# wenbowen123/iros20-6d-pose-tracking

Measured on AMD Instinct MI355X. Metric: RGB-D pair inferences/sec (176x176), higher is better.
Workload: dtype f32; 1 GPU; configs[1]: batch=64 synthetic 176x176 RGB-D pairs per GPU, random-init Se3TrackNet (reference state_dict surface), stage=full; pairs_per_gpu=64, global_batch=64, stage=full, frames=resident in HBM

## Files before the change

### iros20-6d-pose-tracking_amd/csrc/api.cpp

```cpp
#include <cmath>
#include <thread>
#include <type_traits>
#include <cstdio>
#include <cstdlib>
#include <chrono>
#include <cstring>
#include <map>
#include <mutex>
#include <set>
#include <string>
#include <vector>

#include "hip_buffers.h"
#include "pose_align_plan.h"
#include "pose_errors_plan.h"
#include "pose_grid_plan.h"
#include "pose_search_plan.h"
#include "se3tn_internal.h"
#include "tex_pyramid.h"
#include "track_plan.h"
#include "weights.h"

using namespace se3tn;

// ... 17 lines not shown
struct GraphKey {
  const void *A, *B, *trans, *rot, *poseA, *poseB, *blob;
  int layout;
  InferConfig cfg;
  bool operator==(const GraphKey& o) const { return std::memcmp(this, &o, sizeof(GraphKey)) == 0; }
};
struct GraphEntry {
  GraphKey key;
  hipGraphExec_t exec = nullptr;
  InferPlan plan;
};
static_assert(std::is_trivially_copyable<GraphEntry>::value, "the graph cache moves its entries as bytes (GraphKey is compared as bytes)");

struct se3tn_ctx {
  int device = -1, max_batch = 0;
  TensorMap tensors;
  std::vector<float> packed;
  DeviceBuf<float> blob_owned;
  const float* blob = nullptr;
  BlobLayout L;
  DeviceBuf<float> inA, inB;
  DeviceBuf<float> stem;
  DeviceBuf<float> pool, t64, q64;
  DeviceBuf<float> ab, ab_t;
  DeviceBuf<float> head, head_t;
  DeviceBuf<float> head_f;
  unsigned written = 0;
  InferPlan plan;
  DeviceBuf<float> logits;
  DeviceBuf<float> fcpart;
  bool keep_intermediates = false;
  int auto_tile_override[2] = {0, 0};
  int gemmp = -1;
  bool wino_fuse = true;
  DeviceBuf<float> part;
  int tail_parts_ch = 16;
  bool tail_parts = true;
  bool small_kernels = true;
  int wino_min_batch = SE3TN_WINOGRAD_DEFAULT_MIN_BATCH;
  int wino_tile = SE3TN_WINOGRAD_DEFAULT_TILE;
  int wino_tile_derived = 0;
  DeviceBuf<float> wino_u[4];
  DeviceBuf<float> wino_u6[4];
  const float* wino6_blob = nullptr;
  DeviceBuf<float> wino_v, wino_m;
  const float* wino_blob = nullptr;
  int wino64_min_batch = SE3TN_TRUNK_WINOGRAD_DEFAULT_MIN_BATCH;
  int wino64_min_fill = SE3TN_TRUNK_WINOGRAD_DEFAULT_MIN_FILL;
  int num_cus = 256;
  DeviceBuf<float> wino64_u[4];
  const float* wino64_blob = nullptr;
  SplitLayout SL;
  DeviceBuf<float> split_w;
  const float* split_blob = nullptr;
  DeviceBuf<float> wino_us[4];
  DeviceBuf<float> wino_usc[4];
  const float* wino_us_blob = nullptr;
  int wino_us_tile = 0;
  int prec = SE3TN_PREC_F32;
  int offset_rule = SE3TN_OFFSET_RULE_NUMPY1;
  int raster_sub_bits = 4;
  PinnedBuf<uint8_t> trk_host; DeviceBuf<uint8_t> trk_dev; size_t trk_bytes = 0;
  PinnedBuf<uint8_t> trk_out;
  int tb_cap = 0;
  size_t tb_stage_bytes = 0;
  PinnedBuf<uint8_t> tb_inst_host; DeviceBuf<uint8_t> tb_inst_dev;
// ... 268 lines not shown
    d = c->ps_dev.get();
    return SE3TN_OK;
  }
  int upload(size_t bytes) const {
    HIPCHK(hipMemcpyAsync(d, h, bytes, hipMemcpyHostToDevice, st));
    return SE3TN_OK;
  }
  int finish(size_t at, size_t bytes) const {
    HIPCHK(hipMemcpyAsync(h + at, d + at, bytes, hipMemcpyDeviceToHost, st));
    HIPCHK(hipStreamSynchronize(st));
    return SE3TN_OK;
  }
  template <class T> T* dev(size_t at) const { return reinterpret_cast<T*>(d + at); }
};

extern "C" {

const char* se3tn_version(void) { return "se3tracknet-gfx950 0.6.0 (blob v7)"; }
const char* se3tn_last_error(void) { return g_err.c_str(); }

int se3tn_create(int device, int max_batch, se3tn_ctx** out) {
  if (!out || max_batch < 1) return fail(SE3TN_E_ARG, "se3tn_create: bad argument");
  if (max_batch > SE3TN_MAX_BATCH_LIMIT)
    return fail(SE3TN_E_ARG, "se3tn_create: max_batch " + std::to_string(max_batch) + " exceeds SE3TN_MAX_BATCH_LIMIT (" +
                                 std::to_string(SE3TN_MAX_BATCH_LIMIT) + "): run larger sets as several calls");
  se3tn_ctx* c = new se3tn_ctx();
  c->device = device;
  c->max_batch = max_batch;
  c->L = blob_layout();
  c->SL = split_layout();
  if (const char* e = std::getenv("SE3TN_WINOGRAD_AUTO_TILE_AB2")) c->auto_tile_override[0] = (std::atoi(e) == 4 || std::atoi(e) == 6) ? std::atoi(e) : 0;
  if (const char* e = std::getenv("SE3TN_WINOGRAD_AUTO_TILE_HEADS")) c->auto_tile_override[1] = (std::atoi(e) == 4 || std::atoi(e) == 6) ? std::atoi(e) : 0;
  if (const char* e = std::getenv("SE3TN_WINO_GEMMP")) c->gemmp = std::atoi(e) != 0 ? 1 : 0;
  if (const char* e = std::getenv("SE3TN_WINOGRAD_FUSE")) c->wino_fuse = std::atoi(e) != 0;
  if (const char* e = std::getenv("SE3TN_TRUNK_WINOGRAD")) c->wino64_min_batch = std::atoi(e);
  if (const char* e = std::getenv("SE3TN_TRUNK_WINOGRAD_FILL")) c->wino64_min_fill = std::atoi(e);
  for (int i = 0; i < 8; ++i) { c->mean[i] = 0.0; c->stdv[i] = 1.0; }
  if (device >= 0) {
    hipDeviceProp_t prop;
    hipError_t e = hipGetDeviceProperties(&prop, device);
    if (e != hipSuccess) { delete c; return hipfail(e, "hipGetDeviceProperties"); }
    if (std::strncmp(prop.gcnArchName, "gfx950", 6) != 0) {
      std::string a = prop.gcnArchName;
      delete c;
      return fail(SE3TN_E_DEVICE, "device is " + a + ", this library is built for gfx950 only");
    }
    if (prop.multiProcessorCount > 0) c->num_cus = prop.multiProcessorCount;
    e = hipSetDevice(device);
    if (e != hipSuccess) { delete c; return hipfail(e, "hipSetDevice"); }
    const size_t mb = (size_t)max_batch;
    auto padded = [&](int s, int ch) { return (mb * (s + 2) * (s + 2) + PAD_SLACK_PX) * ch; };
    struct { DeviceBuf<float>* p; size_t words; bool zero; } bufs[] = {
        {&c->inA, (mb * IN_P + IN_SLACK_ROWS) * IN_P * 4, true},
        {&c->inB, (mb * IN_P + IN_SLACK_ROWS) * IN_P * 4, true},
        {&c->stem, mb * S1 * S1 * 128, false}, {&c->pool, padded(S2, 128), true},
        {&c->t64, padded(S2, 128), true},      {&c->q64, padded(S2, 128), true},
        {&c->ab, padded(S3, 256), true},       {&c->ab_t, padded(S3, 256), true},
        {&c->head, padded(S4, 1024), true},    {&c->head_t, padded(S4, 1024), true},
        {&c->head_f, padded(S4, 1024), true},
        {&c->logits, mb * 6, true},           {&c->fcpart, mb * 192, true}};
    for (auto& b : bufs) {
      e = b.p->alloc(b.words, b.zero);
      if (e != hipSuccess) { delete c; return hipfail(e, "hipMalloc(workspace)"); }
    }
    e = c->part.alloc((size_t)16 * 1024 * 121 * 16);
    if (e == hipSuccess) e = c->tail_arrive.alloc(c->max_batch, true);
// ... 278 lines not shown
  if (fast) {
    a.fast = 1;
    a.overflow = c->overflow.get();
    a.w = c->split_w.get() + c->SL.conv_ws[r.id];
    a.wscale = c->split_w.get() + c->SL.conv_sc[r.id];
  }
  a.res = tensor_ptr(c, r.res, fast); a.out = tensor_ptr(c, r.out, fast);
  a.part = c->part.get(); a.part_bytes = c->part.count() * sizeof(float);
  a.in_ld = r.in.ld; a.res_ld = r.res.ld; a.out_ld = r.out.ld;
  a.H = r.hin; a.W = r.hin; a.Ho = (r.hin - 1) / r.stride + 1; a.Wo = a.Ho;
  a.M = n * a.Ho * a.Wo;
  a.groups = s.groups;
  a.in_gs = r.in.gs; a.res_gs = r.res.gs; a.out_gs = r.out.gs; a.bias_gs = s.cout;
  a.w_gs = (long long)conv3_words(s.cin, s.cout);
  if (ip) {
    a.per_img = 1;
    std::memcpy(a.img_off, ip->off, sizeof(a.img_off));
  }
}
static void fill_wino_args(se3tn_ctx* c, const ConvRow& r, int tile, int n, const float* W, bool split, WinoArgs& w) {
  const Conv3& s = conv_specs()[r.id];
  const int ws = wino_slot(r.id);
  w = WinoArgs{};
  w.in = tensor_ptr(c, r.in, split); w.bias = W + c->L.conv_b[r.id]; w.res = tensor_ptr(c, r.res, split); w.out = tensor_ptr(c, r.out, split);
  w.U = tile == 6 ? c->wino_u6[ws].get() : c->wino_u[ws].get();
  w.V = c->wino_v.get(); w.Mw = c->wino_m.get();
  w.in_ld = r.in.ld; w.res_ld = r.res.ld; w.out_ld = r.out.ld;
  w.m = tile; w.nf = (tile + 2) * (tile + 2);
  w.H = r.hin; w.W = r.hin; w.th = (r.hin + tile - 1) / tile; w.tw = w.th;
  w.n = n; w.T = n * w.th * w.tw;
  w.C = s.cin; w.Cout = s.cout; w.groups = s.groups;
  w.in_gs = r.in.gs; w.res_gs = r.res.gs; w.out_gs = r.out.gs; w.bias_gs = s.cout;
  w.u_gs = (long long)w.nf * s.cin * s.cout;
  if (split) {
    w.split = 1;
    w.U = c->wino_us[ws].get(); w.uscale = c->wino_usc[ws].get();
    w.overflow = c->overflow.get();
  }
}

static int infer_launch(se3tn_ctx* c, const float* A, const float* B, int n, int layout, float* trans, float* rot,
                        const double* poseA, double* poseB, void* stream);

int se3tn_enable_graphs(se3tn_ctx* c, int on) {
  if (!c || c->device < 0) return fail(SE3TN_E_ARG, "se3tn_enable_graphs: no device context");
  c->use_graphs = on != 0;
  return SE3TN_OK;
}

static int infer_graph_or_launch(se3tn_ctx* c, const float* A, const float* B, int n, int layout, float* trans, float* rot,
                                 const double* poseA, double* poseB, void* stream);

int se3tn_infer(se3tn_ctx* c, const float* A, const float* B, int n, int layout, float* trans, float* rot,
                const double* poseA, double* poseB, void* stream) {
  if (c && c->rearm_counters && c->device >= 0 && !stream_is_capturing((hipStream_t)stream)) {
    if (c->tail_arrive) HIPCHK(hipMemsetAsync(c->tail_arrive.get(), 0, sizeof(int) * c->max_batch, (hipStream_t)stream));
    c->rearm_counters = false;
  }
  const int rc = infer_graph_or_launch(c, A, B, n, layout, trans, rot, poseA, poseB, stream);
  if (rc != SE3TN_OK && rc != SE3TN_E_ARG && rc != SE3TN_E_STATE && c) c->rearm_counters = true;
  return rc;
}

static int infer_graph_or_launch(se3tn_ctx* c, const float* A, const float* B, int n, int layout, float* trans, float* rot,
                                 const double* poseA, double* poseB, void* stream) {
  if (!c || !c->use_graphs || c->prof || stream == nullptr)
// ... 1572 lines not shown
```

### iros20-6d-pose-tracking_amd/csrc/se3tn_internal.h

```cpp
#pragma once
#include <hip/hip_runtime.h>
#include <stddef.h>
#include <stdint.h>

#include "../../include/se3tracknet.h"
#include "infer_plan.h"

namespace se3tn {

struct BlobLayout {
  size_t stem_w;
  size_t stem_b;
  size_t conv_w[NUM_CONV3];
  size_t conv_b[NUM_CONV3];
  size_t fc_w;
  size_t fc_b;
  size_t total;
};

constexpr int HEADER_WORDS = 64;
constexpr uint32_t BLOB_MAGIC = 0x53453354u;
constexpr uint32_t BLOB_VERSION = 7;

struct SplitLayout {
// ... 67 lines not shown
  int groups;
  int in_gs, res_gs, out_gs, bias_gs;
  long long w_gs;
  float* part;
  size_t part_bytes;
  int slices;
  int reserved[2];
  const float* wscale;
  int* overflow;
  int fast;
  int per_img = 0;
  long long img_off[SMALL_MAX_IMG] = {};
};

struct WinoArgs {
  const float* in;
  const float* U;
  const float* bias;
  const float* res;
  float* out;
  float* V;
  float* Mw;
  int in_ld, res_ld, out_ld;
  int H, W;
  int m, nf;
  int th, tw;
  int n, T;
  int C, Cout, groups;
  int in_gs, res_gs, out_gs, bias_gs;
  long long u_gs;
  int split;
  const float* uscale;
  int* overflow;
};

struct TailArgs {
  const float* fc_w;
  const float* fc_b;
  float* logits;
  float* fcpart;
  float* trans;
  float* rot;
  const double* poseA;
  double* poseB;
  double tn, rn;
};

struct CropArgs {
  static constexpr int MAX = 64;
  se3tn_crop c[MAX];
  double mean[8], stdv[8];
  float* out;
  float* out2;
  int n_first;
  int n;
  int padded;
  int split;
  int offset_rule;
  int* overflow;
  const double* norm = nullptr;
  uint8_t* raw_rgb = nullptr;
  uint16_t* raw_depth = nullptr;
};

static_assert(sizeof(CropArgs) <= 4096, "CropArgs travels as kernel arguments: HIP's limit is 4 KB");

// ... 212 lines not shown
```

### iros20-6d-pose-tracking_amd/csrc/wino_mfma.hip

```cpp
#include "mfma_common.h"
#include "pose_device.h"

#ifndef WINO4_VEC
#define WINO4_VEC 2
#endif
#ifndef WINO_MID_CS_AB
#define WINO_MID_CS_AB 32
#endif
#ifndef WINO_MID_CS_H
#define WINO_MID_CS_H 32
#endif

#ifdef SE3TN_GEMMP_TRACE
__device__ unsigned long long se3tn_gemmp_trace[8 * 64 * 5];
extern "C" int se3tn_debug_gemmp_trace(void* host_out, size_t bytes) {
  return (int)hipMemcpyFromSymbol(host_out, HIP_SYMBOL(se3tn_gemmp_trace), bytes, 0, hipMemcpyDeviceToHost);
}
#define GP_STAMP(K, I) if (blockIdx.x == 0 && lane == 0 && (K) < 64) ::se3tn_gemmp_trace[(wid * 64 + (K)) * 5 + (I)] = __builtin_amdgcn_s_memtime();
#else
#define GP_STAMP(K, I)
#endif
#ifdef SE3TN_WG_TRACE
__device__ unsigned long long se3tn_wg_trace[8 * 4096];
extern "C" int se3tn_debug_wg_trace(void* host_out, size_t bytes, int clear) {
  if (clear) {
    void* p = nullptr;
    if (hipGetSymbolAddress(&p, HIP_SYMBOL(se3tn_wg_trace)) != hipSuccess) return 1;
    return (int)hipMemset(p, 0, sizeof(unsigned long long) * 8 * 4096);
  }
  return (int)hipMemcpyFromSymbol(host_out, HIP_SYMBOL(se3tn_wg_trace), bytes, 0, hipMemcpyDeviceToHost);
}
#endif

namespace se3tn {
// ... 59 lines not shown
  const hv h = *reinterpret_cast<const hv*>(p_);
  const hv l = *reinterpret_cast<const hv*>(p_ + 64);
#pragma unroll
  for (int e = 0; e < VEC; ++e) o[e] = (float)h[e] + (float)l[e];
}
template <int VEC>
__device__ __forceinline__ bool store_split_vec(float* base, size_t row, int ld, int c, const float (&v)[VEC]) {
  unsigned char* p_ = reinterpret_cast<unsigned char*>(base) + split_byte_off(row, ld, c);
  typedef _Float16 hv __attribute__((ext_vector_type(VEC)));
  hv h, l;
  bool bad = false;
#pragma unroll
  for (int e = 0; e < VEC; ++e) {
    h[e] = (_Float16)v[e];
    l[e] = (_Float16)(v[e] - (float)h[e]);
    bad |= !(fabsf(v[e]) <= 65000.f);
  }
  *reinterpret_cast<hv*>(p_) = h;
  *reinterpret_cast<hv*>(p_ + 64) = l;
  return bad;
}

struct TileId { int t, cv, n, ty, tx; };
__device__ __forceinline__ TileId tile_of(int idx, int cvn, int th, int tw) {
  TileId r;
  r.cv = idx % cvn; r.t = idx / cvn;
  const int tpi = th * tw;
  r.n = r.t / tpi;
  const int rem = r.t - r.n * tpi;
  r.ty = rem / tw; r.tx = rem - r.ty * tw;
  return r;
}

template <int M, int VEC, int SP = 0>
__global__ __launch_bounds__(256) void wino_input_kernel(const WinoArgs a) {
  constexpr int N = M + 2;
  typedef typename VecT<VEC>::type vec;
  const int cvn = a.C / VEC;
  const int idx = blockIdx.x * 256 + threadIdx.x;
  if (idx >= a.T * cvn) return;
  const int g = blockIdx.y;
  const TileId id = tile_of(idx, cvn, a.th, a.tw);
  const int Hp = a.H + 2, Wp = a.W + 2;
  const float* __restrict__ src = a.in + (size_t)g * a.in_gs + (SP ? 0 : id.cv * VEC);
  float bt[N][N][VEC];
  if constexpr (M == 6) {
    static_assert(SP == 0, "F(6x6) is a float32 path");
#pragma unroll
    for (int s = 0; s < N; ++s) {
      float dc[N][VEC];
      const int X = M * id.tx + s;
#pragma unroll
      for (int r = 0; r < N; ++r) {
        const int Y = M * id.ty + r;
        vec v;
        if (Y < Hp && X < Wp) v = *reinterpret_cast<const vec*>(src + (size_t)((id.n * Hp + Y) * Wp + X) * a.in_ld);
        else __builtin_memset(&v, 0, sizeof(v));
        __builtin_memcpy(dc[r], &v, sizeof(v));
      }
#pragma unroll
      for (int i = 0; i < N; ++i)
#pragma unroll
        for (int e = 0; e < VEC; ++e) {
          float acc = 0.f;
          bool first = true;
#pragma unroll
          for (int r = 0; r < N; ++r) axpy(acc, wino_bt<M>(i, r), dc[r][e], first);
          bt[i][s][e] = acc;
        }
    }
  } else {
  float d[N][N][VEC];
#pragma unroll
  for (int r = 0; r < N; ++r)
#pragma unroll
    for (int s = 0; s < N; ++s) {
      const int Y = M * id.ty + r, X = M * id.tx + s;
      if (SP) {
        if (Y < Hp && X < Wp) load_split_vec<VEC>(src, (size_t)((id.n * Hp + Y) * Wp + X), a.in_ld, id.cv * VEC, d[r][s]);
        else for (int e = 0; e < VEC; ++e) d[r][s][e] = 0.f;
        continue;
      }
      vec v;
      if (Y < Hp && X < Wp) v = *reinterpret_cast<const vec*>(src + (size_t)((id.n * Hp + Y) * Wp + X) * a.in_ld);
      else __builtin_memset(&v, 0, sizeof(v));
      __builtin_memcpy(d[r][s], &v, sizeof(v));
    }
#pragma unroll
  for (int i = 0; i < N; ++i)
#pragma unroll
    for (int s = 0; s < N; ++s)
#pragma unroll
      for (int e = 0; e < VEC; ++e) {
        float acc = 0.f;
        bool first = true;
#pragma unroll
        for (int r = 0; r < N; ++r) axpy(acc, wino_bt<M>(i, r), d[r][s][e], first);
        bt[i][s][e] = acc;
      }
  }
  float* __restrict__ dst = a.V + ((size_t)g * a.nf * a.T + id.t) * a.C + (SP ? 0 : id.cv * VEC);
  const size_t fs = (size_t)a.T * a.C;
  bool bad = false;
#pragma unroll
  for (int i = 0; i < N; ++i)
#pragma unroll
    for (int j = 0; j < N; ++j) {
      float o[VEC];
#pragma unroll
      for (int e = 0; e < VEC; ++e) {
        float acc = 0.f;
        bool first = true;
#pragma unroll
        for (int s = 0; s < N; ++s) axpy(acc, wino_bt<M>(j, s), bt[i][s][e], first);
        o[e] = acc;
      }
      if (SP) {
        bad |= store_split_vec<VEC>(dst + (size_t)(N * i + j) * fs, 0, a.C, id.cv * VEC, o);
        continue;
      }
      vec v;
      __builtin_memcpy(&v, o, sizeof(v));
      *reinterpret_cast<vec*>(dst + (size_t)(N * i + j) * fs) = v;
    }
  if (SP && bad) atomicOr(a.overflow, 1);
}

template <int M, int VEC, int EPI, int SP = 0>
__global__ __launch_bounds__(256) void wino_output_kernel(const WinoArgs a) {
  constexpr int N = M + 2;
  typedef typename VecT<VEC>::type vec;
  const int cvn = a.Cout / VEC;
  const int idx = blockIdx.x * 256 + threadIdx.x;
  if (idx >= a.T * cvn) return;
  const int g = blockIdx.y;
  const TileId id = tile_of(idx, cvn, a.th, a.tw);
  const int Hp = a.H + 2, Wp = a.W + 2;
  const float* __restrict__ src = a.Mw + ((size_t)g * a.nf * a.T + id.t) * a.Cout + id.cv * VEC;
  const size_t fs = (size_t)a.T * a.Cout;
  float rr[M][M][VEC];
  if constexpr (EPI == 1 && SP == 0) {
    const float* __restrict__ res0 = a.res + (size_t)g * a.res_gs + id.cv * VEC;
#pragma unroll
    for (int i = 0; i < M; ++i)
#pragma unroll
      for (int j = 0; j < M; ++j) {
        int oy = M * id.ty + i, ox = M * id.tx + j;
        oy = oy < a.H ? oy : a.H - 1; ox = ox < a.W ? ox : a.W - 1;
        const vec v = *reinterpret_cast<const vec*>(res0 + (size_t)((id.n * Hp + oy + 1) * Wp + ox + 1) * a.res_ld);
        __builtin_memcpy(rr[i][j], &v, sizeof(v));
      }
  }
  float u[M][N][VEC];
#pragma unroll
  for (int s = 0; s < N; ++s) {
    float m[N][VEC];
#pragma unroll
    for (int r = 0; r < N; ++r) {
      const vec v = *reinterpret_cast<const vec*>(src + (size_t)(N * r + s) * fs);
      __builtin_memcpy(m[r], &v, sizeof(v));
    }
#pragma unroll
    for (int i = 0; i < M; ++i)
#pragma unroll
      for (int e = 0; e < VEC; ++e) {
        float acc = 0.f;
        bool first = true;
#pragma unroll
        for (int r = 0; r < N; ++r) axpy(acc, wino_at<M>(i, r), m[r][e], first);
        u[i][s][e] = acc;
      }
  }
  float b[VEC];
  {
    const vec v = *reinterpret_cast<const vec*>(a.bias + (size_t)g * a.bias_gs + id.cv * VEC);
    __builtin_memcpy(b, &v, sizeof(v));
  }
  const float* __restrict__ res = (EPI == 1) ? a.res + (size_t)g * a.res_gs + (SP ? 0 : id.cv * VEC) : nullptr;
  float* __restrict__ out = a.out + (size_t)g * a.out_gs + (SP ? 0 : id.cv * VEC);
  bool bad = false;
  if constexpr (SP == 0) __builtin_amdgcn_s_waitcnt(0x0F70);
#pragma unroll
  for (int i = 0; i < M; ++i)
#pragma unroll
    for (int j = 0; j < M; ++j) {
      const int oy = M * id.ty + i, ox = M * id.tx + j;
      if (oy >= a.H || ox >= a.W) continue;
      const size_t pix = (size_t)((id.n * Hp + oy + 1) * Wp + ox + 1);
      float r[VEC];
      if (EPI == 1) {
        if (SP) {
          load_split_vec<VEC>(res, pix, a.res_ld, id.cv * VEC, r);
// ... 39 lines not shown
  double gg[N][3];
#pragma unroll
  for (int i = 0; i < N; ++i)
#pragma unroll
    for (int s = 0; s < 3; ++s) gg[i][s] = wino_g<M>(i, 0) * g[0][s] + wino_g<M>(i, 1) * g[1][s] + wino_g<M>(i, 2) * g[2][s];
  const size_t fs = (size_t)cout * 32;
  float* dst = U + ((size_t)ch * N * N * cout + co) * 32 + k;
#pragma unroll
  for (int i = 0; i < N; ++i)
#pragma unroll
    for (int j = 0; j < N; ++j)
      dst[(size_t)(N * i + j) * fs] = (float)(gg[i][0] * wino_g<M>(j, 0) + gg[i][1] * wino_g<M>(j, 1) + gg[i][2] * wino_g<M>(j, 2));
}

template <int CIN, int WM, int WN, int PT, int CT, int MM = MM_F32>
__global__ __launch_bounds__(256, 2) void wino_gemm_kernel(const WinoArgs a) {
  constexpr int BM = WM * PT * 32, BN = WN * CT * 32;
  constexpr int NCH = CIN / 32;
  constexpr int BUF = (BM + BN) * 32;
  static_assert(WM * WN == 4, "4 waves");
  extern __shared__ __attribute__((aligned(16))) float smem[];

  const int tid = threadIdx.x;
  const int lane = tid & 63;
  const int wid = __builtin_amdgcn_readfirstlane(tid >> 6);
  const int wm = wid / WN, wn = wid % WN;
  const int l31 = lane & 31, hh = lane >> 5;

  const int panels = a.Cout / BN, mtiles = (a.T + BM - 1) / BM;
  const int nt = blockIdx.x % panels, rest = blockIdx.x / panels;
  const int mt = rest % mtiles, b = rest / mtiles;
  const int g = b / a.nf, f = b - g * a.nf;
  const int m0 = mt * BM, n0 = nt * BN;
  const float* __restrict__ Vb = a.V + (size_t)b * a.T * CIN;
  const float* __restrict__ Ub = a.U + (size_t)g * a.u_gs + ((size_t)f * a.Cout + n0) * 32;
  const int mlast = a.T - 1;

  const int r0 = tid >> 3;
  const int c4 = (tid & 7) ^ ((r0 >> 1) & 7);
  unsigned pvoff[BM / 32];
#pragma unroll
  for (int j = 0; j < BM / 32; ++j) pvoff[j] = (unsigned)((min(m0 + r0 + 32 * j, mlast) * CIN + c4 * 4) * 4);
  const unsigned wvoff = (unsigned)((r0 * 32 + c4 * 4) * 4);
  const unsigned lds0 = __builtin_amdgcn_readfirstlane(lds_addr_of(smem));

#define ISSUE_TILE(CH, BUFI)                                                                         \
  {                                                                                                  \
    const float* pb_ = Vb + (CH) * 32;                                                               \
    const unsigned lb_ = lds0 + (unsigned)(((BUFI) * BUF + wid * 256) * 4);                          \
    _Pragma("unroll") for (int j_ = 0; j_ < BM / 32; ++j_) glds16<0>(pb_, pvoff[j_], lb_ + j_ * 4096); \
    const float* tb_ = Ub + (size_t)(CH) * a.nf * a.Cout * 32;                                       \
    _Pragma("unroll") for (int j_ = 0; j_ < BN / 32; ++j_)                                           \
        glds16<0>(tb_ + 1024 * j_, wvoff, lb_ + BM * 128 + j_ * 4096);                               \
  }

  const int X = (l31 >> 1) & 7;
  const int lo = (hh ^ (X & 1)) * 4, xk = X >> 1;
  const int fo0 = ((0 ^ xk) << 3) + lo, fo1 = ((1 ^ xk) << 3) + lo, fo2 = ((2 ^ xk) << 3) + lo,
            fo3 = ((3 ^ xk) << 3) + lo;

  f32x16 acc[PT][CT];
#pragma unroll
  for (int i = 0; i < PT; ++i)
#pragma unroll
    for (int j = 0; j < CT; ++j)
#pragma unroll
      for (int e = 0; e < 16; ++e) acc[i][j][e] = 0.f;

#ifdef SE3TN_WG_TRACE
// ... 48 lines not shown
    for (int j = 0; j < CT; ++j)
#pragma unroll
      for (int q = 0; q < 4; ++q) {
        const int c = n0 + (wn * CT + j) * 32 + q * 8 + hh * 4;
        float4 v = make_float4(acc[i][j][4 * q + 0], acc[i][j][4 * q + 1], acc[i][j][4 * q + 2], acc[i][j][4 * q + 3]);
        if (MM == MM_F16X3) {
          const float4 w = *reinterpret_cast<const float4*>(wsc + c);
          v.x *= w.x; v.y *= w.y; v.z *= w.z; v.w *= w.w;
        }
        *reinterpret_cast<float4*>(Mb + (size_t)m * a.Cout + c) = v;
      }
  }
#ifdef SE3TN_WG_TRACE
  if (tid == 0 && blockIdx.x < 4096) ::se3tn_wg_trace[blockIdx.x * 8 + 5] = __builtin_amdgcn_s_memrealtime();
#endif
}

template <int CIN>
__global__ __launch_bounds__(512, 2) void wino_gemmp_kernel(const WinoArgs a, int total_tiles) {
  constexpr int BM = 128, BN = 256;
  constexpr int WN = 4, PT = 2, CT = 2;
  constexpr int VP = BM / 64;
  constexpr int NCH = CIN / 32;
  constexpr int BUF = (BM + BN) * 32;
  static_assert(NCH % 2 == 0, "the double buffer's parity must be the same at every tile start");
  extern __shared__ __attribute__((aligned(16))) float smem[];

  const int tid = threadIdx.x;
  const int lane = tid & 63;
  const int wid = __builtin_amdgcn_readfirstlane(tid >> 6);
  const int wm = wid / WN, wn = wid % WN;
  const int l31 = lane & 31, hh = lane >> 5;
  const int panels = a.Cout / BN, mtiles = (a.T + BM - 1) / BM, tpp = panels * mtiles;
  const int mlast = a.T - 1;

  const int r0 = tid >> 3;
  const int c4 = (tid & 7) ^ ((r0 >> 1) & 7);
  const unsigned wvoff = (unsigned)((r0 * 32 + c4 * 4) * 4);
  const unsigned lds0 = __builtin_amdgcn_readfirstlane(lds_addr_of(smem));

  auto decode = [&](int v, int& b, int& m0, int& n0) {
    const int xcd = v & 7, s = v >> 3;
    const int q = s / tpp, r = s - q * tpp;
    b = q * 8 + xcd;
    n0 = (r % panels) * BN;
    m0 = (r / panels) * BM;
  };
  const float* Vb;
  const float* Ub;
  unsigned pvoff[VP];
  auto set_tile = [&](int b, int m0, int n0) {
    const int g = b / a.nf, f = b - g * a.nf;
    Vb = a.V + (size_t)b * a.T * CIN;
    Ub = a.U + (size_t)g * a.u_gs + ((size_t)f * a.Cout + n0) * 32;
#pragma unroll
    for (int j = 0; j < VP; ++j) pvoff[j] = (unsigned)((min(m0 + r0 + 64 * j, mlast) * CIN + c4 * 4) * 4);
  };
#define ISSUE_TILEP(CH, BUFI)                                                                        \
  {                                                                                                  \
    const float* pb_ = Vb + (CH) * 32;                                                               \
    const unsigned lb_ = lds0 + (unsigned)(((BUFI) * BUF + wid * 256) * 4);                          \
    _Pragma("unroll") for (int j_ = 0; j_ < VP; ++j_) glds16<0>(pb_, pvoff[j_], lb_ + j_ * 8192);     \
    const float* tb_ = Ub + (size_t)(CH) * a.nf * a.Cout * 32;                                       \
    _Pragma("unroll") for (int j_ = 0; j_ < 4; ++j_) glds16<0>(tb_ + 2048 * j_, wvoff, lb_ + BM * 128 + j_ * 8192); \
  }

  const int X = (l31 >> 1) & 7;
  const int lo = (hh ^ (X & 1)) * 4, xk = X >> 1;
  const int fo0 = ((0 ^ xk) << 3) + lo, fo1 = ((1 ^ xk) << 3) + lo, fo2 = ((2 ^ xk) << 3) + lo, fo3 = ((3 ^ xk) << 3) + lo;

  f32x16 acc[PT][CT];
#pragma unroll
  for (int i = 0; i < PT; ++i)
#pragma unroll
    for (int j = 0; j < CT; ++j)
#pragma unroll
      for (int e = 0; e < 16; ++e) acc[i][j][e] = 0.f;

  int v = blockIdx.x;
  if (v >= total_tiles) return;
  int b, m0, n0;
  decode(v, b, m0, n0);
  set_tile(b, m0, n0);
  ISSUE_TILEP(0, 0)
  wait_dma_and_barrier();

  int kstep_ = 0;
  (void)kstep_;
  while (true) {
    const int vn = v + gridDim.x;
    const bool more = vn < total_tiles;
    const int cb = b, cm0 = m0, cn0 = n0;
#pragma unroll 1
    for (int ch = 0; ch < NCH; ++ch) {
      const int buf = ch & 1;
      GP_STAMP(kstep_, 0)
      if (ch + 1 < NCH) {
        ISSUE_TILEP(ch + 1, buf ^ 1)
      } else if (more) {
        decode(vn, b, m0, n0);
        set_tile(b, m0, n0);
        ISSUE_TILEP(0, buf ^ 1)
      }
      GP_STAMP(kstep_, 1)
      const float* pP = smem + buf * BUF + (wm * PT * 32 + l31) * 32;
      const float* pW = smem + buf * BUF + (BM + wn * CT * 32 + l31) * 32;
#define FOG(G) ((G) == 0 ? fo0 : (G) == 1 ? fo1 : (G) == 2 ? fo2 : fo3)
#define PXF(G) *reinterpret_cast<const float4*>(pP + i * 1024 + FOG(G))
#define WTF(G) *reinterpret_cast<const float4*>(pW + j * 1024 + FOG(G))
      SE3TN_MMA_GROUP(PT, CT, PXF(0), WTF(0))
      SE3TN_MMA_GROUP(PT, CT, PXF(1), WTF(1))
      SE3TN_MMA_GROUP(PT, CT, PXF(2), WTF(2))
      SE3TN_MMA_GROUP(PT, CT, PXF(3), WTF(3))
#undef PXF
#undef WTF
#undef FOG
      GP_STAMP(kstep_, 2)
      if (ch + 1 < NCH || more) {
        asm volatile("s_waitcnt vmcnt(0)" ::: "memory");
        GP_STAMP(kstep_, 3)
        __syncthreads();
      }
      GP_STAMP(kstep_, 4)
      ++kstep_;
    }
    float* __restrict__ Mb = a.Mw + (size_t)cb * a.T * a.Cout;
#pragma unroll
    for (int i = 0; i < PT; ++i) {
      const int m = cm0 + (wm * PT + i) * 32 + l31;
#pragma unroll
      for (int j = 0; j < CT; ++j)
#pragma unroll
        for (int q = 0; q < 4; ++q) {
          const int c = cn0 + (wn * CT + j) * 32 + q * 8 + hh * 4;
          if (m <= mlast)
            *reinterpret_cast<float4*>(Mb + (size_t)m * a.Cout + c) =
                make_float4(acc[i][j][4 * q + 0], acc[i][j][4 * q + 1], acc[i][j][4 * q + 2], acc[i][j][4 * q + 3]);
#pragma unroll
          for (int e = 0; e < 4; ++e) acc[i][j][4 * q + e] = 0.f;
        }
    }
    if (!more) break;
    v = vn;
  }
#undef ISSUE_TILEP
}

template <> struct VecT<1> { typedef float type; };

template <int M, int TH, int CS, int VEC, int SP = 0>
__global__ __launch_bounds__(((TH * TH * (CS / VEC) + 63) / 64) * 64) void wino_mid_kernel(const WinoArgs a, float* __restrict__ keep) {
  constexpr int N = M + 2, HP = M * TH + 2, NT = TH * TH, CP = CS / VEC, ITEMS = NT * CP;
  typedef typename VecT<VEC>::type vec;
  static_assert(SP == 0 || (M == 4 && VEC == 2), "the f16x3 blocks are F(4x4) with channel pairs");
  extern __shared__ __attribute__((aligned(16))) float act[];
  const int n = blockIdx.x, c0 = blockIdx.y * CS, g = blockIdx.z;
  const int tid = threadIdx.x;
  for (int i = tid; i < HP * HP * CS / 4; i += blockDim.x) reinterpret_cast<float4*>(act)[i] = make_float4(0.f, 0.f, 0.f, 0.f);
  __syncthreads();
  const int tile = tid / CP, cp = tid - tile * CP;
  const int ty = tile / TH, tx = tile - ty * TH;
  const bool active = tid < ITEMS;
  const int t = n * NT + tile;
  const int Hp = a.H + 2, Wp = a.W + 2;
  if (active) {
    const float* __restrict__ src = a.Mw + ((size_t)g * a.nf * a.T + t) * a.Cout + c0 + cp * VEC;
    const size_t fs = (size_t)a.T * a.Cout;
    float u[M][N][VEC];
#pragma unroll
    for (int s = 0; s < N; ++s) {
      float m[N][VEC];
#pragma unroll
      for (int r = 0; r < N; ++r) {
        const vec v = *reinterpret_cast<const vec*>(src + (size_t)(N * r + s) * fs);
        __builtin_memcpy(m[r], &v, sizeof(v));
      }
#pragma unroll
      for (int i = 0; i < M; ++i)
#pragma unroll
        for (int e = 0; e < VEC; ++e) {
          float acc = 0.f;
          bool first = true;
#pragma unroll
          for (int r = 0; r < N; ++r) axpy(acc, wino_at<M>(i, r), m[r][e], first);
          u[i][s][e] = acc;
        }
    }
    float b[VEC];
    {
      const vec v = *reinterpret_cast<const vec*>(a.bias + (size_t)g * a.bias_gs + c0 + cp * VEC);
      __builtin_memcpy(b, &v, sizeof(v));
    }
    float* __restrict__ kp = keep ? keep + (size_t)g * a.out_gs + c0 + cp * VEC : nullptr;
#pragma unroll
    for (int i = 0; i < M; ++i)
#pragma unroll
      for (int j = 0; j < M; ++j) {
        const int oy = M * ty + i, ox = M * tx + j;
        if (oy >= a.H || ox >= a.W) continue;
        float o[VEC];
#pragma unroll
        for (int e = 0; e < VEC; ++e) {
          float acc = 0.f;
          bool first = true;
#pragma unroll
          for (int s = 0; s < N; ++s) axpy(acc, wino_at<M>(j, s), u[i][s][e], first);
          acc += b[e];
          o[e] = fmaxf(acc, 0.f);
        }
        vec v;
        __builtin_memcpy(&v, o, sizeof(v));
        *reinterpret_cast<vec*>(act + ((oy + 1) * HP + ox + 1) * CS + cp * VEC) = v;
        if (kp) *reinterpret_cast<vec*>(kp + (size_t)((n * Hp + oy + 1) * Wp + ox + 1) * a.out_ld) = v;
      }
  }
  __syncthreads();
  if (active) {
    float bt[N][N][VEC];
#pragma unroll
    for (int s = 0; s < N; ++s) {
      float d[N][VEC];
#pragma unroll
      for (int r = 0; r < N; ++r) {
        const vec v = *reinterpret_cast<const vec*>(act + ((M * ty + r) * HP + M * tx + s) * CS + cp * VEC);
        __builtin_memcpy(d[r], &v, sizeof(v));
      }
#pragma unroll
      for (int i = 0; i < N; ++i)
#pragma unroll
        for (int e = 0; e < VEC; ++e) {
          float acc = 0.f;
          bool first = true;
#pragma unroll
          for (int r = 0; r < N; ++r) axpy(acc, wino_bt<M>(i, r), d[r][e], first);
          bt[i][s][e] = acc;
        }
    }
    float* __restrict__ dst = a.V + ((size_t)g * a.nf * a.T + t) * a.C + (SP ? 0 : c0 + cp * VEC);
    const size_t fs = (size_t)a.T * a.C;
    bool bad = false;
#pragma unroll
    for (int i = 0; i < N; ++i)
#pragma unroll
      for (int j = 0; j < N; ++j) {
        float o[VEC];
#pragma unroll
        for (int e = 0; e < VEC; ++e) {
          float acc = 0.f;
          bool first = true;
#pragma unroll
          for (int s = 0; s < N; ++s) axpy(acc, wino_bt<M>(j, s), bt[i][s][e], first);
          o[e] = acc;
        }
        if constexpr (SP != 0) {
          bad |= store_split_vec<VEC>(dst + (size_t)(N * i + j) * fs, 0, a.C, c0 + cp * VEC, o);
        } else {
          vec v;
          __builtin_memcpy(&v, o, sizeof(v));
          *reinterpret_cast<vec*>(dst + (size_t)(N * i + j) * fs) = v;
        }
      }
    if (SP && bad) atomicOr(a.overflow, 1);
  }
}

__device__ __forceinline__ float wave_sum64(float v) {
#pragma unroll
  for (int o = 32; o > 0; o >>= 1) v += __shfl_xor(v, o, 64);
  return v;
}

template <int M, int TH, int CS, int SP = 0>
__global__ __launch_bounds__(((TH * TH * (CS / 2) + 63) / 64) * 64) void wino_tail_kernel(const WinoArgs a, float* __restrict__ keep,
                                                                                         const float* __restrict__ fc_w,
                                                                                         float* __restrict__ fcpart) {
  constexpr int N = M + 2, NT = TH * TH, CP = CS / 2, ITEMS = NT * CP;
  static_assert(SP == 0 || M == 4, "the f16x3 blocks are F(4x4)");
  static_assert(CP == 32, "the FC partials are reduced inside one half-wave");
  __shared__ float red[NT][CP][2];
  const int n = blockIdx.x, sl = blockIdx.y, g = blockIdx.z, tid = threadIdx.x;
  const int tile = tid / CP, cp = tid - tile * CP;
  const int c = sl * CS + cp * 2;
  const int Hp = a.H + 2, Wp = a.W + 2;
  if (tid < ITEMS) {
    const int ty = tile / TH, tx = tile - ty * TH;
    const size_t fs = (size_t)a.T * a.Cout;
    const float* __restrict__ src = a.Mw + ((size_t)g * a.nf * a.T + n * NT + tile) * a.Cout + c;
    const float* __restrict__ res = a.res + (size_t)g * a.res_gs + (SP ? 0 : c);
    float* __restrict__ kp = keep ? keep + (size_t)g * a.out_gs + c : nullptr;
    const float2 b = *reinterpret_cast<const float2*>(a.bias + (size_t)g * a.bias_gs + c);
    float2 rr[M][M];
    if constexpr (SP == 0) {
#pragma unroll
      for (int i = 0; i < M; ++i)
#pragma unroll
        for (int j = 0; j < M; ++j) {
          int oy = M * ty + i, ox = M * tx + j;
          oy = oy < a.H ? oy : a.H - 1; ox = ox < a.W ? ox : a.W - 1;
          rr[i][j] = *reinterpret_cast<const float2*>(res + (size_t)((n * Hp + oy + 1) * Wp + ox + 1) * a.res_ld);
        }
    }
    float u[M][N][2];
#pragma unroll
    for (int s = 0; s < N; ++s) {
      float m[N][2];
#pragma unroll
      for (int r = 0; r < N; ++r) {
        const float2 v = *reinterpret_cast<const float2*>(src + (size_t)(N * r + s) * fs);
        m[r][0] = v.x; m[r][1] = v.y;
      }
#pragma unroll
      for (int i = 0; i < M; ++i)
#pragma unroll
        for (int e = 0; e < 2; ++e) {
          float acc = 0.f;
          bool first = true;
#pragma unroll
          for (int r = 0; r < N; ++r) axpy(acc, wino_at<M>(i, r), m[r][e], first);
          u[i][s][e] = acc;
        }
    }
    float sum[2] = {0.f, 0.f};
#pragma unroll
    for (int i = 0; i < M; ++i)
#pragma unroll
      for (int j = 0; j < M; ++j) {
        const int oy = M * ty + i, ox = M * tx + j;
        if (oy >= a.H || ox >= a.W) continue;
        const size_t pix = (size_t)((n * Hp + oy + 1) * Wp + ox + 1);
        float2 r;
        if (SP) {
          float rr[2];
          load_split_vec<2>(res, pix, a.res_ld, c, rr);
          r = make_float2(rr[0], rr[1]);
        } else {
          r = rr[i][j];
        }
        float o[2];
#pragma unroll
        for (int e = 0; e < 2; ++e) {
          float acc = 0.f;
// ... 211 lines not shown
```

Baseline: 41850 pairs/s.

## Skip Winograd frequency rows that only touch padded edge tiles

Adds a WinoRows indexing scheme that, when the tile grid overhangs the image, drops the last-row/column frequency components of edge tiles whose contributions fall entirely outside the output. The input transform stops storing them, the batched GEMM compacts row counts per frequency and skips empty M-tiles, and the output transforms substitute zeros for them. This cuts GEMM work and V/M traffic for layers where H is not a multiple of the tile size. In exchange it adds per-element index arithmetic and branching in the transforms and a more complex persistent-tile scheduler.

```diff
diff --git a/iros20-6d-pose-tracking_amd/csrc/api.cpp b/iros20-6d-pose-tracking_amd/csrc/api.cpp
--- a/iros20-6d-pose-tracking_amd/csrc/api.cpp
+++ b/iros20-6d-pose-tracking_amd/csrc/api.cpp
@@ -73,6 +73,7 @@
   bool keep_intermediates = false;
   int auto_tile_override[2] = {0, 0};
   int gemmp = -1;
+  bool wino_skip_edge = true;
   bool wino_fuse = true;
   DeviceBuf<float> part;
   int tail_parts_ch = 16;
@@ -407,6 +408,7 @@
   if (const char* e = std::getenv("SE3TN_WINOGRAD_AUTO_TILE_AB2")) c->auto_tile_override[0] = (std::atoi(e) == 4 || std::atoi(e) == 6) ? std::atoi(e) : 0;
   if (const char* e = std::getenv("SE3TN_WINOGRAD_AUTO_TILE_HEADS")) c->auto_tile_override[1] = (std::atoi(e) == 4 || std::atoi(e) == 6) ? std::atoi(e) : 0;
   if (const char* e = std::getenv("SE3TN_WINO_GEMMP")) c->gemmp = std::atoi(e) != 0 ? 1 : 0;
+  if (const char* e = std::getenv("SE3TN_WINO_SKIP_EDGE")) c->wino_skip_edge = std::atoi(e) != 0;
   if (const char* e = std::getenv("SE3TN_WINOGRAD_FUSE")) c->wino_fuse = std::atoi(e) != 0;
   if (const char* e = std::getenv("SE3TN_TRUNK_WINOGRAD")) c->wino64_min_batch = std::atoi(e);
   if (const char* e = std::getenv("SE3TN_TRUNK_WINOGRAD_FILL")) c->wino64_min_fill = std::atoi(e);
@@ -751,6 +753,7 @@
   w.C = s.cin; w.Cout = s.cout; w.groups = s.groups;
   w.in_gs = r.in.gs; w.res_gs = r.res.gs; w.out_gs = r.out.gs; w.bias_gs = s.cout;
   w.u_gs = (long long)w.nf * s.cin * s.cout;
+  w.skip_edge = c->wino_skip_edge ? 1 : 0;
   if (split) {
     w.split = 1;
     w.U = c->wino_us[ws].get(); w.uscale = c->wino_usc[ws].get();
diff --git a/iros20-6d-pose-tracking_amd/csrc/se3tn_internal.h b/iros20-6d-pose-tracking_amd/csrc/se3tn_internal.h
--- a/iros20-6d-pose-tracking_amd/csrc/se3tn_internal.h
+++ b/iros20-6d-pose-tracking_amd/csrc/se3tn_internal.h
@@ -123,6 +123,7 @@
   int split;
   const float* uscale;
   int* overflow;
+  int skip_edge;
 };
 
 struct TailArgs {
diff --git a/iros20-6d-pose-tracking_amd/csrc/wino_mfma.hip b/iros20-6d-pose-tracking_amd/csrc/wino_mfma.hip
--- a/iros20-6d-pose-tracking_amd/csrc/wino_mfma.hip
+++ b/iros20-6d-pose-tracking_amd/csrc/wino_mfma.hip
@@ -1,5 +1,6 @@
 #include "mfma_common.h"
 #include "pose_device.h"
+#include "wino_rows.h"
 
 #ifndef WINO4_VEC
 #define WINO4_VEC 2
@@ -125,6 +126,8 @@
   return r;
 }
 
+__device__ __forceinline__ WinoRows wino_rows(const WinoArgs& a, int M) { return WinoRows(M, a.H, a.W, a.th, a.tw, a.n, a.skip_edge != 0); }
+
 template <int M, int VEC, int SP = 0>
 __global__ __launch_bounds__(256) void wino_input_kernel(const WinoArgs a) {
   constexpr int N = M + 2;
@@ -134,6 +137,7 @@
   if (idx >= a.T * cvn) return;
   const int g = blockIdx.y;
   const TileId id = tile_of(idx, cvn, a.th, a.tw);
+  const WinoRows wr = wino_rows(a, M);
   const int Hp = a.H + 2, Wp = a.W + 2;
   const float* __restrict__ src = a.in + (size_t)g * a.in_gs + (SP ? 0 : id.cv * VEC);
   float bt[N][N][VEC];
@@ -192,13 +196,16 @@
         bt[i][s][e] = acc;
       }
   }
-  float* __restrict__ dst = a.V + ((size_t)g * a.nf * a.T + id.t) * a.C + (SP ? 0 : id.cv * VEC);
+  float* __restrict__ dst = a.V + (size_t)g * a.nf * a.T * a.C;
+  const unsigned ch0 = SP ? 0u : (unsigned)(id.cv * VEC);
   const size_t fs = (size_t)a.T * a.C;
   bool bad = false;
 #pragma unroll
   for (int i = 0; i < N; ++i)
 #pragma unroll
     for (int j = 0; j < N; ++j) {
+      const bool keep = wr.needed(i, j, id.ty, id.tx);
+      float* __restrict__ dp = dst + (size_t)(N * i + j) * fs + ((unsigned)(wr.row(i, j, id.n, id.ty, id.tx) * a.C) + ch0);
       float o[VEC];
 #pragma unroll
       for (int e = 0; e < VEC; ++e) {
@@ -209,12 +216,12 @@
         o[e] = acc;
       }
       if (SP) {
-        bad |= store_split_vec<VEC>(dst + (size_t)(N * i + j) * fs, 0, a.C, id.cv * VEC, o);
+        if (keep) bad |= store_split_vec<VEC>(dp, 0, a.C, id.cv * VEC, o);
         continue;
       }
       vec v;
       __builtin_memcpy(&v, o, sizeof(v));
-      *reinterpret_cast<vec*>(dst + (size_t)(N * i + j) * fs) = v;
+      if (keep) *reinterpret_cast<vec*>(dp) = v;
     }
   if (SP && bad) atomicOr(a.overflow, 1);
 }
@@ -228,8 +235,10 @@
   if (idx >= a.T * cvn) return;
   const int g = blockIdx.y;
   const TileId id = tile_of(idx, cvn, a.th, a.tw);
+  const WinoRows wr = wino_rows(a, M);
   const int Hp = a.H + 2, Wp = a.W + 2;
-  const float* __restrict__ src = a.Mw + ((size_t)g * a.nf * a.T + id.t) * a.Cout + id.cv * VEC;
+  const float* __restrict__ src = a.Mw + (size_t)g * a.nf * a.T * a.Cout;
+  const unsigned ch0 = (unsigned)(id.cv * VEC);
   const size_t fs = (size_t)a.T * a.Cout;
   float rr[M][M][VEC];
   if constexpr (EPI == 1 && SP == 0) {
@@ -250,7 +259,9 @@
     float m[N][VEC];
 #pragma unroll
     for (int r = 0; r < N; ++r) {
-      const vec v = *reinterpret_cast<const vec*>(src + (size_t)(N * r + s) * fs);
+      vec v;
+      if (wr.needed(r, s, id.ty, id.tx)) v = *reinterpret_cast<const vec*>(src + (size_t)(N * r + s) * fs + ((unsigned)(wr.row(r, s, id.n, id.ty, id.tx) * a.Cout) + ch0));
+      else __builtin_memset(&v, 0, sizeof(v));
       __builtin_memcpy(m[r], &v, sizeof(v));
     }
 #pragma unroll
@@ -356,9 +367,10 @@
   const int mt = rest % mtiles, b = rest / mtiles;
   const int g = b / a.nf, f = b - g * a.nf;
   const int m0 = mt * BM, n0 = nt * BN;
+  const int mlast = wino_rows(a, a.m).rows(f) - 1;
+  if (m0 > mlast) return;
   const float* __restrict__ Vb = a.V + (size_t)b * a.T * CIN;
   const float* __restrict__ Ub = a.U + (size_t)g * a.u_gs + ((size_t)f * a.Cout + n0) * 32;
-  const int mlast = a.T - 1;
 
   const int r0 = tid >> 3;
   const int c4 = (tid & 7) ^ ((r0 >> 1) & 7);
@@ -473,7 +485,7 @@
   const int wm = wid / WN, wn = wid % WN;
   const int l31 = lane & 31, hh = lane >> 5;
   const int panels = a.Cout / BN, mtiles = (a.T + BM - 1) / BM, tpp = panels * mtiles;
-  const int mlast = a.T - 1;
+  const WinoRows wr = wino_rows(a, a.m);
 
   const int r0 = tid >> 3;
   const int c4 = (tid & 7) ^ ((r0 >> 1) & 7);
@@ -487,10 +499,20 @@
     n0 = (r % panels) * BN;
     m0 = (r / panels) * BM;
   };
+  auto next_slot = [&](int v, int& b, int& m0, int& n0, int& mlast) -> int {
+    for (; v < total_tiles; v += gridDim.x) {
+      decode(v, b, m0, n0);
+      const int f = b % a.nf;
+      const int i = a.m == 6 ? f >> 3 : a.m == 2 ? f >> 2 : f / 6;
+      mlast = wr.rows(i, f - (a.m + 2) * i) - 1;
+      if (m0 <= mlast) break;
+    }
+    return v;
+  };
   const float* Vb;
   const float* Ub;
   unsigned pvoff[VP];
-  auto set_tile = [&](int b, int m0, int n0) {
+  auto set_tile = [&](int b, int m0, int n0, int mlast) {
     const int g = b / a.nf, f = b - g * a.nf;
     Vb = a.V + (size_t)b * a.T * CIN;
     Ub = a.U + (size_t)g * a.u_gs + ((size_t)f * a.Cout + n0) * 32;
@@ -518,30 +540,32 @@
 #pragma unroll
       for (int e = 0; e < 16; ++e) acc[i][j][e] = 0.f;
 
-  int v = blockIdx.x;
+  int b = 0, m0 = 0, n0 = 0, mlast = 0;
+  int v = next_slot(blockIdx.x, b, m0, n0, mlast);
   if (v >= total_tiles) return;
-  int b, m0, n0;
-  decode(v, b, m0, n0);
-  set_tile(b, m0, n0);
+  set_tile(b, m0, n0, mlast);
   ISSUE_TILEP(0, 0)
   wait_dma_and_barrier();
 
   int kstep_ = 0;
   (void)kstep_;
   while (true) {
-    const int vn = v + gridDim.x;
-    const bool more = vn < total_tiles;
-    const int cb = b, cm0 = m0, cn0 = n0;
+    const int cb = b, cm0 = m0, cn0 = n0, cmlast = mlast;
+    int vn = v;
+    bool more = false;
 #pragma unroll 1
     for (int ch = 0; ch < NCH; ++ch) {
       const int buf = ch & 1;
       GP_STAMP(kstep_, 0)
       if (ch + 1 < NCH) {
         ISSUE_TILEP(ch + 1, buf ^ 1)
-      } else if (more) {
-        decode(vn, b, m0, n0);
-        set_tile(b, m0, n0);
-        ISSUE_TILEP(0, buf ^ 1)
+      } else {
+        vn = next_slot(v + gridDim.x, b, m0, n0, mlast);
+        more = vn < total_tiles;
+        if (more) {
+          set_tile(b, m0, n0, mlast);
+          ISSUE_TILEP(0, buf ^ 1)
+        }
       }
       GP_STAMP(kstep_, 1)
       const float* pP = smem + buf * BUF + (wm * PT * 32 + l31) * 32;
@@ -574,7 +598,7 @@
 #pragma unroll
         for (int q = 0; q < 4; ++q) {
           const int c = cn0 + (wn * CT + j) * 32 + q * 8 + hh * 4;
-          if (m <= mlast)
+          if (m <= cmlast)
             *reinterpret_cast<float4*>(Mb + (size_t)m * a.Cout + c) =
                 make_float4(acc[i][j][4 * q + 0], acc[i][j][4 * q + 1], acc[i][j][4 * q + 2], acc[i][j][4 * q + 3]);
 #pragma unroll
@@ -602,10 +626,11 @@
   const int tile = tid / CP, cp = tid - tile * CP;
   const int ty = tile / TH, tx = tile - ty * TH;
   const bool active = tid < ITEMS;
-  const int t = n * NT + tile;
+  const WinoRows wr = wino_rows(a, M);
   const int Hp = a.H + 2, Wp = a.W + 2;
   if (active) {
-    const float* __restrict__ src = a.Mw + ((size_t)g * a.nf * a.T + t) * a.Cout + c0 + cp * VEC;
+    const float* __restrict__ src = a.Mw + (size_t)g * a.nf * a.T * a.Cout;
+    const unsigned ch0 = (unsigned)(c0 + cp * VEC);
     const size_t fs = (size_t)a.T * a.Cout;
     float u[M][N][VEC];
 #pragma unroll
@@ -613,7 +638,9 @@
       float m[N][VEC];
 #pragma unroll
       for (int r = 0; r < N; ++r) {
-        const vec v = *reinterpret_cast<const vec*>(src + (size_t)(N * r + s) * fs);
+        vec v;
+        if (wr.needed(r, s, ty, tx)) v = *reinterpret_cast<const vec*>(src + (size_t)(N * r + s) * fs + ((unsigned)(wr.row(r, s, n, ty, tx) * a.Cout) + ch0));
+        else __builtin_memset(&v, 0, sizeof(v));
         __builtin_memcpy(m[r], &v, sizeof(v));
       }
 #pragma unroll
@@ -677,13 +704,16 @@
           bt[i][s][e] = acc;
         }
     }
-    float* __restrict__ dst = a.V + ((size_t)g * a.nf * a.T + t) * a.C + (SP ? 0 : c0 + cp * VEC);
+    float* __restrict__ dst = a.V + (size_t)g * a.nf * a.T * a.C;
+    const unsigned vch0 = SP ? 0u : (unsigned)(c0 + cp * VEC);
     const size_t fs = (size_t)a.T * a.C;
     bool bad = false;
 #pragma unroll
     for (int i = 0; i < N; ++i)
 #pragma unroll
       for (int j = 0; j < N; ++j) {
+        const bool keepv = wr.needed(i, j, ty, tx);
+        float* __restrict__ dp = dst + (size_t)(N * i + j) * fs + ((unsigned)(wr.row(i, j, n, ty, tx) * a.C) + vch0);
         float o[VEC];
 #pragma unroll
         for (int e = 0; e < VEC; ++e) {
@@ -694,11 +724,11 @@
           o[e] = acc;
         }
         if constexpr (SP != 0) {
-          bad |= store_split_vec<VEC>(dst + (size_t)(N * i + j) * fs, 0, a.C, c0 + cp * VEC, o);
+          if (keepv) bad |= store_split_vec<VEC>(dp, 0, a.C, c0 + cp * VEC, o);
         } else {
           vec v;
           __builtin_memcpy(&v, o, sizeof(v));
-          *reinterpret_cast<vec*>(dst + (size_t)(N * i + j) * fs) = v;
+          if (keepv) *reinterpret_cast<vec*>(dp) = v;
         }
       }
     if (SP && bad) atomicOr(a.overflow, 1);
@@ -725,8 +755,9 @@
   const int Hp = a.H + 2, Wp = a.W + 2;
   if (tid < ITEMS) {
     const int ty = tile / TH, tx = tile - ty * TH;
+    const WinoRows wr = wino_rows(a, M);
     const size_t fs = (size_t)a.T * a.Cout;
-    const float* __restrict__ src = a.Mw + ((size_t)g * a.nf * a.T + n * NT + tile) * a.Cout + c;
+    const float* __restrict__ src = a.Mw + (size_t)g * a.nf * a.T * a.Cout;
     const float* __restrict__ res = a.res + (size_t)g * a.res_gs + (SP ? 0 : c);
     float* __restrict__ kp = keep ? keep + (size_t)g * a.out_gs + c : nullptr;
     const float2 b = *reinterpret_cast<const float2*>(a.bias + (size_t)g * a.bias_gs + c);
@@ -747,7 +778,8 @@
       float m[N][2];
 #pragma unroll
       for (int r = 0; r < N; ++r) {
-        const float2 v = *reinterpret_cast<const float2*>(src + (size_t)(N * r + s) * fs);
+        float2 v = make_float2(0.f, 0.f);
+        if (wr.needed(r, s, ty, tx)) v = *reinterpret_cast<const float2*>(src + (size_t)(N * r + s) * fs + (unsigned)(wr.row(r, s, n, ty, tx) * a.Cout + c));
         m[r][0] = v.x; m[r][1] = v.y;
       }
 #pragma unroll
diff --git a/iros20-6d-pose-tracking_amd/csrc/wino_rows.h b/iros20-6d-pose-tracking_amd/csrc/wino_rows.h
--- /dev/null
+++ b/iros20-6d-pose-tracking_amd/csrc/wino_rows.h
@@ -0,0 +1,26 @@
+#pragma once
+
+#if defined(__HIPCC__)
+#define SE3TN_WR_HD __host__ __device__ __forceinline__
+#else
+#define SE3TN_WR_HD inline
+#endif
+
+namespace se3tn {
+
+struct WinoRows {
+  int m, th, tw, n;
+  bool drop_y, drop_x;
+  SE3TN_WR_HD constexpr WinoRows(int m_, int H, int W, int th_, int tw_, int n_, bool skip)
+      : m(m_), th(th_), tw(tw_), n(n_), drop_y(skip && th_ * m_ > H), drop_x(skip && tw_ * m_ > W) {}
+  SE3TN_WR_HD constexpr int th_f(int i) const { return th - ((drop_y && i == m + 1) ? 1 : 0); }
+  SE3TN_WR_HD constexpr int tw_f(int j) const { return tw - ((drop_x && j == m + 1) ? 1 : 0); }
+  SE3TN_WR_HD constexpr bool needed(int i, int j, int ty, int tx) const {
+    return !(i == m + 1 && drop_y && ty == th - 1) && !(j == m + 1 && drop_x && tx == tw - 1);
+  }
+  SE3TN_WR_HD constexpr int rows(int i, int j) const { return n * th_f(i) * tw_f(j); }
+  SE3TN_WR_HD constexpr int rows(int f) const { return rows(f / (m + 2), f % (m + 2)); }
+  SE3TN_WR_HD constexpr int row(int i, int j, int img, int ty, int tx) const { return (img * th_f(i) + ty) * tw_f(j) + tx; }
+};
+
+}
```

Measured after the change: 41950 pairs/s, median of 6. No clear change (+0.3%).
